# xiexh20/CHORE

Measured on AMD Instinct MI355X. Metric: query-points/sec (HGFilters encode + 20k-pt MLP field query per 512x512 image), higher is better.
Workload: dtype fp16x3; 1 GPU; BASELINE configs[1]: encode 4x(5,512,512) + query 4x20000 points per GPU per step; images_per_gpu=4, points_per_image=20000, batches_in_flight=2

## Files before the change

chore_amd/csrc/conv_mw.hip:

```cpp
#include "conv_common.h"
#include <cstdio>
#include <cstdlib>
#include <cstring>
#include <type_traits>

using namespace conv_detail;

#ifndef MW_DBG
#define MW_DBG 0
#endif

#ifdef MW_STAMPS
__device__ unsigned long long g_mw_stamps[2048 * 8];
#define MWSTAMP(i) do { if (threadIdx.x == 0 && blockIdx.x < 2048) g_mw_stamps[blockIdx.x * 8 + (i)] = wall_clock64(); } while (0)
extern "C" int chore_debug_mw_stamps(unsigned long long* out, int n) {
    return (int)hipMemcpyFromSymbol(out, HIP_SYMBOL(g_mw_stamps), sizeof(unsigned long long) * (n < 2048 * 8 ? n : 2048 * 8));
}
#else
#define MWSTAMP(i) do { } while (0)
#endif

namespace {

constexpr int PTW = 32;
constexpr int MWT = 256;

template <int TAPS, int TH_, int NT_, int TPS_, int NSLOT_, bool X3_, int WPL_> struct MGeo {
    static constexpr int TH = TH_, NT = NT_, TPS = TPS_, NSLOT = NSLOT_;
    static constexpr int PAD = (TAPS == 9) ? 1 : 0;
    static constexpr int PW = PTW + 2 * PAD, PH = TH + 2 * PAD, ROWS = PH * PW;
    static constexpr int RB = X3_ ? 144 : 80;
    static constexpr int PATCHB = (ROWS + 1) * RB;
    static constexpr int KROWS = TAPS / TPS;
    static constexpr int NB = NT / 32;
    static constexpr int SB1 = TPS * KGC * NB * 1024;
    static constexpr int SBYTES = WPL_ * SB1;
    static constexpr int NBW = NT >= 128 ? 2 : (NT == 64 ? (TH_ >= 4 ? 2 : 1) : 1);
    static constexpr int WAVES_N = NB / NBW, WAVES_M = 4 / WAVES_N, MB = TH / WAVES_M;
    static constexpr int SCR_LD = NT + 4;
    static constexpr int G8 = NT / 8;
    static constexpr int NU = TH * PTW * G8 / MWT;
    static constexpr bool CROSS = NSLOT >= 3 && KROWS > 1;
    static constexpr size_t main_bytes(int Cin) { return (size_t)2 * PATCHB + (size_t)NSLOT * SBYTES + (size_t)Cin * 8 + 16; }
    static constexpr int NROW = MWT / G8;
    static constexpr int NSEG = 4 * NT >= MWT ? 1 : MWT / (4 * NT);
    static constexpr size_t stat_bytes(int kinds) { return (size_t)(NROW + NSEG) * kinds * NT * 4; }
    static constexpr size_t scr_bytes() { return (size_t)TH * PTW * SCR_LD * 4; }
    static constexpr size_t epi_bytes() {
        size_t m = scr_bytes();
        if (stat_bytes(4) > m) m = stat_bytes(4);
        if (stat_bytes(6) > m) m = stat_bytes(6);
        return m;
    }
    static size_t smem_bytes(int Cin) { return main_bytes(Cin) > epi_bytes() ? main_bytes(Cin) : epi_bytes(); }
    static_assert(MB >= 1 && WAVES_M * MB == TH, "tile rows must divide over the waves");
    static_assert(NU >= 1, "epilogue units");
    static_assert((SBYTES / 16) % MWT == 0, "a K-step's weights: whole vectors per thread");
};

__host__ __device__ constexpr int mw_next_use(int k, int j, int UP, int KROWS, int RPS, int NVP) {
    for (int d = UP; d < KROWS; d += UP)
        if (((k + d) % KROWS) * RPS + j < NVP) return k + d;
    return k + KROWS;
}

typedef float f32x2 __attribute__((ext_vector_type(2)));
typedef _Float16 f16x2_t __attribute__((ext_vector_type(2)));
__device__ __forceinline__ unsigned cvt_pk_f16(float a, float b) {
    const f16x2_t h = {(_Float16)a, (_Float16)b};
    return __builtin_bit_cast(unsigned, h);
}
template <int HI> __device__ __forceinline__ float sub_half(float y, unsigned h) {
    float r;
    if constexpr (HI) asm("v_fma_mix_f32 %0, -%1, 1.0, %2 op_sel:[1,0,0] op_sel_hi:[1,0,0]" : "=v"(r) : "v"(h), "v"(y));
    else asm("v_fma_mix_f32 %0, -%1, 1.0, %2 op_sel:[0,0,0] op_sel_hi:[1,0,0]" : "=v"(r) : "v"(h), "v"(y));
    return r;
}

__device__ __forceinline__ void wg_barrier_mw() {
    asm volatile("s_waitcnt lgkmcnt(0)" ::: "memory");
    __builtin_amdgcn_s_barrier();
    asm volatile("" ::: "memory");
    __builtin_amdgcn_sched_barrier(0);
}

template <typename T, int TAPS, int TH_, int NT_, int TPS_, int NSLOT_, bool GN, bool SC, bool POOL = false>
__global__ __launch_bounds__(MWT, 1) void conv_mw_kernel(ConvArgs a) {
    if constexpr (IS_X3<T> || IS_H16<T>) f16_saturate_mode();
    constexpr bool BF = std::is_same<T, bf16_t>::value;
    static_assert(IS_X3<T> || IS_H16<T> || BF, "conv_mw_kernel: fp16 x 3, fp16 or bf16 operands");
    constexpr bool X3 = IS_X3<T>;
    constexpr int WPL = BF ? 1 : 2;
    using ST = typename std::conditional<X3, float, unsigned short>::type;
    constexpr int LVI = X3 ? 2 : 1;
    using G = MGeo<TAPS, TH_, NT_, TPS_, NSLOT_, X3, WPL>;
    constexpr int NSLOT = G::NSLOT;
    constexpr int TH = G::TH, NT = G::NT, TPS = G::TPS, PAD = G::PAD, PW = G::PW, ROWS = G::ROWS, RB = G::RB;
    constexpr int PATCHB = G::PATCHB, KROWS = G::KROWS, SB1 = G::SB1, SBYTES = G::SBYTES;
    constexpr int NBW = G::NBW, WAVES_N = G::WAVES_N, MB = G::MB, SCR_LD = G::SCR_LD, G8 = G::G8, NU = G::NU;
    constexpr bool CROSS = G::CROSS;
    constexpr int KGE = 16, CC = 32;
    constexpr int NTASK = ROWS * 4;
    constexpr int NVP = (NTASK + MWT - 1) / MWT;
    constexpr int RPS = KROWS > 1 ? (NVP + KROWS - 2) / (KROWS > 1 ? KROWS - 1 : 1) : NVP;
    constexpr int SVEC = SBYTES / 16, SBV = SVEC / MWT, SV1 = SB1 / 16;
    constexpr int NKS = TPS * KGC;
    constexpr int UP = KROWS == 9 ? 3 : KROWS;
    static_assert(KROWS % UP == 0 && NKS % 2 == 0, "register-set rotation / fragment double buffer");

    extern __shared__ __attribute__((aligned(16))) char smem[];
    char* patch = smem;
    char* bst = smem + 2 * PATCHB;
    float* ss_lds = (float*)(bst + NSLOT * SBYTES);

    const int tid = threadIdx.x, lane = tid & 63;
    const int wid = __builtin_amdgcn_readfirstlane(tid >> 6);
    MWSTAMP(0);
    float in_mul = 1.f, in_inv = 1.f;
    if constexpr (X3 && SC) x3_in_scale(a.in_amax, in_mul, in_inv);
    const int wn = wid % WAVES_N, wm = wid / WAVES_N;
    const int tiles_x = (a.W + PTW - 1) / PTW;
    const int ntn = a.Cout / NT, tiles = tiles_x * ((a.H + TH - 1) / TH);
    int lid = blockIdx.x;
    {
        const int nwg = gridDim.x, q = nwg >> 3, r = nwg & 7, xcd = lid & 7;
        lid = (xcd < r ? xcd * (q + 1) : r * (q + 1) + (xcd - r) * q) + (lid >> 3);
    }
    const int n_tile = lid % ntn, tileb = lid / ntn, tile = tileb % tiles, b = tileb / tiles;
    const int ty0 = (tile / tiles_x) * TH, tx0 = (tile % tiles_x) * PTW;
    const int Cin = a.in.C;
    const int NKG = Cin / KGE, NB = a.Cout / 32;
    const int NCH = Cin / CC;
    const ST* in_b = (const ST*)a.in.p + (size_t)b * a.H * a.W * a.in.cs + a.in.co;

    const int crot = (tile * 5 + n_tile * 3) % NCH;
    auto chunk_of = [&](int ci) -> int { int x = ci + crot; return x >= NCH ? x - NCH : x; };

    const int tv = tid & 3;
    int toff[NVP];
    int trow[NVP];
#pragma unroll
    for (int m = 0; m < NVP; ++m) {
        const int row = (tid >> 2) + (MWT / 4) * m;
// ... 112 lines not shown
            for (int j = 0; j < SBV; ++j) wpro[u][j] = wb[woff[j]];
        }
        __builtin_amdgcn_sched_barrier(0);
        if (tid < Cin) {
            float sc = 1.f, sh = 0.f;
            if constexpr (GN) {
                double t[2];
#pragma unroll
                for (int k = 0; k < 2; ++k) {
                    const long long top = st_hi[k] + (long long)(st_lo[k] >> 32);
                    t[k] = ((double)top * 0x1p32 + (double)(st_lo[k] & 0xffffffffull)) * 0x1p-40;
                }
                const double n = (double)(a.H * a.W) * gs_in;
                const double mean = t[0] / n;
                double var = t[1] / n - mean * mean;
                if (var < 0.0) var = 0.0;
                const float rstd = 1.0f / sqrtf((float)var + 1e-5f);
                sc = rstd * gam;
                sh = bet - (float)mean * sc;
            }
            ss_lds[4 * (tid >> 1) + (tid & 1)] = sc;
            ss_lds[4 * (tid >> 1) + 2 + (tid & 1)] = sh;
        }
#pragma unroll
        for (int m = 0; m < NVP; ++m) {
            const int row = (tid >> 2) + (MWT / 4) * m;
            if (toff[m] < 0 && row < ROWS) {
                const u32x4 z = {0u, 0u, 0u, 0u};
#pragma unroll
                for (int pbuf = 0; pbuf < 2; ++pbuf) {
                    char* d = patch + pbuf * PATCHB + row * RB + tv * 16;
                    *(u32x4*)d = z;
                    if constexpr (X3) *(u32x4*)(d + 64) = z;
                }
            }
        }
        wg_barrier_mw();
        f32x2 sc[4], sh[4];
        load_ss(sc, sh, c00);
#pragma unroll
        for (int m = 0; m < NVP; ++m) put_task(p0[m], toff[m], sc, sh, trow[m], 0);
#pragma unroll
        for (int u = 0; u < NPRO; ++u)
#pragma unroll
            for (int j = 0; j < SBV; ++j) *(u32x4*)(bst + u * SBYTES + (tid + j * MWT) * 16) = wpro[u][j];
    }

    const float ASCALE = BF ? 1.0f : (SC ? in_inv / (float)(1 << X3_WSHIFT) : 1.0f / (float)(1 << X3_WSHIFT));
    const int g8 = tid % G8;
    const int nv = n_tile * NT + g8 * 8;
    const size_t img = (size_t)b * a.H * a.W;
    const ST* res_p = a.res.p ? (const ST*)a.res.p + img * a.res.cs + a.res.co + nv : nullptr;

    u32x4 rq[NU][LVI];
    auto fetch_res = [&]() {
#pragma unroll
        for (int j = 0; j < NU; ++j) {
            const int p = (tid + MWT * j) / G8;
            const int y = ty0 + p / PTW, x = tx0 + p % PTW;
            const bool ok = (y < a.H) && (x < a.W);
            const size_t pix = (size_t)y * a.W + x;
            const u32x4 z = {0u, 0u, 0u, 0u};
#pragma unroll
            for (int k = 0; k < LVI; ++k) rq[j][k] = (res_p && ok) ? *((const u32x4*)(res_p + pix * a.res.cs) + k) : z;
        }
    };

    f32x16 acc[MB][NBW];
#pragma unroll
    for (int m = 0; m < MB; ++m)
#pragma unroll
        for (int q = 0; q < NBW; ++q)
#pragma unroll
            for (int r = 0; r < 16; ++r) acc[m][q][r] = 0.f;

    u32x4 pset[UP][RPS][LVI], wset[SBV];
    auto task_of = [&](int k, int j) -> int { return k * RPS + j; };
#pragma unroll
    for (int k = 0; k < UP; ++k)
#pragma unroll
        for (int j = 0; j < RPS; ++j)
            if (task_of(k, j) < NVP) load_task(pset[k][j], toff[task_of(k, j)], chunk_of(NCH > 1 ? 1 : 0) * CC);
    {
        constexpr int u = NSLOT - 1;
        const int uc = u / KROWS < NCH ? u / KROWS : NCH - 1;
        const u32x4* wb = w_of(uc, u % KROWS);
#pragma unroll
        for (int j = 0; j < SBV; ++j) wset[j] = wb[woff[j]];
    }
    const int half = lane >> 5, px = lane & 31;
    const char* a_ptr = patch + ((wm * MB) * PW + px) * RB + 16 * half;
    const char* b_ptr = bst + (wn * NBW) * 1024 + lane * 16;
    u32x4 af[2][MB], afl[2][MB], bf[2][NBW], bfl[2][NBW];
    auto load_frag = [&](int fs, int pbuf, int krow, int slot, int ks) {
        const char* bs = b_ptr + slot * SBYTES;
        const char* ar = a_ptr + pbuf * PATCHB + ((TPS == 3) ? (krow * PW) * RB : ((TPS == 1 && TAPS == 9) ? ((krow / 3) * PW + krow % 3) * RB : 0));
        const int t = ks / KGC, kg = ks % KGC;
        const int ky = (TPS == 9) ? t / 3 : 0, kx = (TPS == 9) ? t % 3 : t;
        if constexpr ((MW_DBG & 8) != 0) return;
#pragma unroll
        for (int q = 0; q < NBW; ++q) bf[fs][q] = *(const u32x4*)(bs + ((t * KGC + kg) * (NT / 32) + q) * 1024);
        if constexpr (X3) {
#pragma unroll
            for (int m = 0; m < MB; ++m) afl[fs][m] = *(const u32x4*)(ar + ((m + ky) * PW + kx) * RB + 64 + kg * 32);
        }
#pragma unroll
        for (int m = 0; m < MB; ++m) af[fs][m] = *(const u32x4*)(ar + ((m + ky) * PW + kx) * RB + kg * 32);
        if constexpr (WPL == 2) {
#pragma unroll
            for (int q = 0; q < NBW; ++q) bfl[fs][q] = *(const u32x4*)(bs + SB1 + ((t * KGC + kg) * (NT / 32) + q) * 1024);
        }
    };
    constexpr int NRD = (X3 ? 2 : 1) * MB + WPL * NBW, NMF = (X3 ? 3 : WPL) * MB * NBW;
    int slot = 0;
    wg_barrier_mw();
    MWSTAMP(1);
    load_frag(0, 0, 0, 0, 0);
// ... 53 lines not shown
                                                                               __builtin_bit_cast(f16x8_t, bf[ks & 1][q]), acc[m][q], 0, 0, 0);
                }
                if constexpr (BF) {
#pragma unroll
                    for (int m = 0; m < MB; ++m)
#pragma unroll
                        for (int q = 0; q < NBW; ++q)
                            acc[m][q] = __builtin_amdgcn_mfma_f32_32x32x16_bf16(__builtin_bit_cast(bf16x8_t, af[ks & 1][m]),
                                                                                __builtin_bit_cast(bf16x8_t, bf[ks & 1][q]), acc[m][q], 0, 0, 0);
                } else {
#pragma unroll
                    for (int m = 0; m < MB; ++m)
#pragma unroll
                        for (int q = 0; q < NBW; ++q)
                            acc[m][q] = __builtin_amdgcn_mfma_f32_32x32x16_f16(__builtin_bit_cast(f16x8_t, af[ks & 1][m]),
                                                                               __builtin_bit_cast(f16x8_t, bfl[ks & 1][q]), acc[m][q], 0, 0, 0);
#pragma unroll
                    for (int m = 0; m < MB; ++m)
#pragma unroll
                        for (int q = 0; q < NBW; ++q)
                            acc[m][q] = __builtin_amdgcn_mfma_f32_32x32x16_f16(__builtin_bit_cast(f16x8_t, af[ks & 1][m]),
                                                                               __builtin_bit_cast(f16x8_t, bf[ks & 1][q]), acc[m][q], 0, 0, 0);
                }
#pragma unroll
                for (int i = 0; i < NMF; ++i) {
                    __builtin_amdgcn_sched_group_barrier(0x008, 1, 0);
                    if (pre && i < NRD) __builtin_amdgcn_sched_group_barrier(0x100, 1, 0);
                    __builtin_amdgcn_sched_group_barrier(0x002, 3, 0);
                    __builtin_amdgcn_sched_group_barrier(0x020, 1, 0);
                    __builtin_amdgcn_sched_group_barrier(0x200, 1, 0);
                }
                __builtin_amdgcn_sched_barrier(0);
            }
            if constexpr ((MW_DBG & 16) == 0) wg_barrier_mw();
            if (!CROSS && !lastk) {
                load_frag(0, k + 1 < KROWS ? pb : pb ^ 1, (k + 1) % KROWS, nslot, 0);
                __builtin_amdgcn_sched_barrier(0);
            }
            slot = nslot;
        }
    };
    {
        int c = 0;
#pragma unroll 1
        for (; c + 1 < NCH; ++c) chunk_body(c, std::true_type{}, std::false_type{});
        chunk_body(c, std::false_type{}, std::true_type{});
    }

    MWSTAMP(2);
    if constexpr ((MW_DBG & 32) != 0) {
        if (a.dbg == 12345) a.bias = (const float*)&acc[0][0];
        return;
    }
    float* scr = (float*)smem;
#pragma unroll
    for (int q = 0; q < NBW; ++q) {
        const int ch = (wn * NBW + q) * 32 + px;
        const float bias = a.bias ? a.bias[n_tile * NT + ch] : 0.f;
#pragma unroll
        for (int m = 0; m < MB; ++m)
#pragma unroll
            for (int r = 0; r < 16; ++r)
                scr[((wm * MB + m) * PTW + mfma32_row(r, half)) * SCR_LD + ch] = acc[m][q][r] * ASCALE + bias;
    }
    wg_barrier_mw();
    MWSTAMP(3);

    static_assert(!POOL || (IS_X3<T> && !SC), "the pooled output: fp32 tensors of the forward pass");
    ST* out_p = (!POOL || a.out.p) ? (ST*)a.out.p + img * a.out.cs + a.out.co + nv : nullptr;
    ST* raw_p = a.raw.p ? (ST*)a.raw.p + img * a.raw.cs + a.raw.co + nv : nullptr;
    using ET = typename std::conditional<X3, float, typename std::conditional<BF, bf16_t, h16_t>::type>::type;
    constexpr bool do_pool = POOL;
    const bool want_stats = a.st_raw || a.st_out || (do_pool && a.st_pool);
    f32x2 sr[4], qr[4], so[4], qo[4];
#pragma unroll
    for (int e = 0; e < 4; ++e) { sr[e] = qr[e] = so[e] = qo[e] = f32x2{0.f, 0.f}; }
#pragma unroll
    for (int j = 0; j < NU; ++j) {
        const int p = (tid + MWT * j) / G8;
        const int y = ty0 + p / PTW, x = tx0 + p % PTW;
        float f[8];
        {
            const f32x4 lo = *(const f32x4*)(scr + p * SCR_LD + g8 * 8), hi = *(const f32x4*)(scr + p * SCR_LD + g8 * 8 + 4);
            f[0] = lo[0]; f[1] = lo[1]; f[2] = lo[2]; f[3] = lo[3]; f[4] = hi[0]; f[5] = hi[1]; f[6] = hi[2]; f[7] = hi[3];
        }
        if (y < a.H && x < a.W) {
            const size_t pix = (size_t)y * a.W + x;
            if (raw_p) {
                float g[8];
#pragma unroll
                for (int e = 0; e < 8; ++e) g[e] = f[e];
                store8<ET>((ET*)(raw_p + pix * a.raw.cs), g);
                if (want_stats) {
#pragma unroll
                    for (int e = 0; e < 4; ++e) {
                        const f32x2 v = {g[2 * e], g[2 * e + 1]};
                        sr[e] += v;
                        qr[e] = __builtin_elementwise_fma(v, v, qr[e]);
                    }
                }
            }
            if (res_p) {
#pragma unroll
                for (int k = 0; k < 4; ++k) {
                    if constexpr (X3) { f[k] += __uint_as_float(rq[j][0][k]); f[4 + k] += __uint_as_float(rq[j][LVI - 1][k]); }
                    else if constexpr (BF) {
// ... 35 lines not shown
                const int pu = tid + MWT * j;
                const int pp = pu / G8, py = pp / (PTW / 2), pxx = pp % (PTW / 2);
                const int oy = (ty0 >> 1) + py, ox = (tx0 >> 1) + pxx;
                if (pu < NPU && oy < OH && ox < OW) {
                    const float* c0 = scr + ((2 * py) * PTW + 2 * pxx) * SCR_LD + g8 * 8;
                    float v[8];
#pragma unroll
                    for (int hv = 0; hv < 2; ++hv) {
                        const f32x4 va = *(const f32x4*)(c0 + 4 * hv), vb = *(const f32x4*)(c0 + SCR_LD + 4 * hv);
                        const f32x4 vc = *(const f32x4*)(c0 + PTW * SCR_LD + 4 * hv), vd = *(const f32x4*)(c0 + (PTW + 1) * SCR_LD + 4 * hv);
                        const f32x4 r = (((va + vb) + vc) + vd) * 0.25f;
                        v[4 * hv] = r[0]; v[4 * hv + 1] = r[1]; v[4 * hv + 2] = r[2]; v[4 * hv + 3] = r[3];
                    }
                    store8<float>(pool_p + ((size_t)oy * OW + ox) * a.pool.cs, v);
#pragma unroll
                    for (int e = 0; e < 4; ++e) {
                        const f32x2 t = {v[2 * e], v[2 * e + 1]};
                        sp[e] += t;
                        qp[e] = __builtin_elementwise_fma(t, t, qp[e]);
                    }
                }
            }
        }
    }

    MWSTAMP(4);
    auto reduce_stats = [&](auto kinds_t) {
        constexpr int KINDS = decltype(kinds_t)::value;
        constexpr int RL = KINDS * NT, NROW = G::NROW, NSEG = G::NSEG, RPSEG = NROW / NSEG;
        static_assert(RPSEG * NSEG == NROW, "statistics reduction geometry");
        static_assert((size_t)(NROW + NSEG) * RL * 4 <= G::epi_bytes(), "statistics reduction scratch");
        wg_barrier_mw();
        float* part = (float*)smem;
        float* red = part + NROW * RL;
        {
            float* pr = part + (tid / G8) * RL + g8 * 8;
            auto park = [&](float* q, const f32x2 (&v)[4]) {
                *(f32x4*)q = f32x4{v[0][0], v[0][1], v[1][0], v[1][1]};
                *(f32x4*)(q + 4) = f32x4{v[2][0], v[2][1], v[3][0], v[3][1]};
            };
            park(pr, sr); park(pr + NT, qr); park(pr + 2 * NT, so); park(pr + 3 * NT, qo);
            if constexpr (KINDS == 6) { park(pr + 4 * NT, sp); park(pr + 5 * NT, qp); }
        }
        wg_barrier_mw();
        for (int cs = tid; cs < NSEG * RL; cs += MWT) {
            const int col = cs % RL, seg = cs / RL;
            const float* pc = part + (seg * RPSEG) * RL + col;
            float t = 0.f;
#pragma unroll
            for (int r = 0; r < RPSEG; ++r) t += pc[r * RL];
            red[seg * RL + col] = t;
        }
        wg_barrier_mw();
        if (tid < NT) {
            const int cg = n_tile * NT + tid;
#pragma unroll
            for (int k = 0; k < KINDS / 2; ++k) {
                GroupStat* st = k == 0 ? a.st_raw : (k == 1 ? a.st_out : a.st_pool);
                if (!st) continue;
                const int gs = (k == 0 ? a.st_raw_C : (k == 1 ? a.st_out_C : a.st_pool_C)) / GN_GROUPS;
                const int co = k == 0 ? a.st_raw_co : (k == 1 ? a.st_out_co : a.st_pool_co);
                float t1 = 0.f, t2 = 0.f;
#pragma unroll
                for (int g = 0; g < NSEG; ++g) { t1 += red[g * RL + (2 * k) * NT + tid]; t2 += red[g * RL + (2 * k + 1) * NT + tid]; }
                const float s1 = group_lane_sum(t1, gs), s2 = group_lane_sum(t2, gs);
                GroupStat* o = st + (size_t)b * GN_GROUPS + (co + cg) / gs;
                if (tid % gs == 0) stat_add(&o->sum, act_hi_cells(a.B), s1);
                if (tid % gs == (gs > 1 ? 1 : 0)) stat_add(&o->sq, act_hi_cells(a.B), s2);
            }
        }
    };
    if (want_stats) {
        reduce_stats(std::integral_constant<int, POOL ? 6 : 4>{});
    }
    MWSTAMP(5);
}

template <typename T, int TAPS, int TH, int NT, int TPS, int NSLOT, bool GN, bool SC, bool POOL = false>
int launch_mw_t(chore_handle* h, const ConvArgs& a, hipStream_t s) {
    using G = MGeo<TAPS, TH, NT, TPS, NSLOT, IS_X3<T>, std::is_same<T, bf16_t>::value ? 1 : 2>;
    size_t smem = G::smem_bytes(a.in.C);
    const size_t lds_cu = chore_lds_per_cu(h);
    if (smem > lds_cu) CHORE_FAIL(h, CHORE_EINVAL, "conv_mw: %zu bytes of LDS, the CU has %zu", smem, lds_cu);
    smem = lds_cu;
    const int tiles = ((a.W + PTW - 1) / PTW) * ((a.H + TH - 1) / TH);
    dim3 grid(tiles * (a.Cout / NT) * a.B);
    return CHORE_LAUNCH(h, s, (conv_mw_kernel<T, TAPS, TH, NT, TPS, NSLOT, GN, SC, POOL>), grid, dim3(MWT), chore_lds(smem, lds_cu), a);
}

}

int conv_mw_fill(int asked) {
    static const int env = getenv("CHORE_CONV_MW_FILL") ? atoi(getenv("CHORE_CONV_MW_FILL")) : 0;
    const int v = env > 0 ? env : asked;
    return v > 0 ? v : 256;
}
bool conv_mw_on(int dtype, int taps) {
    static const char* env = getenv("CHORE_CONV_MW");
    if (env && env[0] == '0') return false;
    return dtype == CHORE_F16X3 && taps == 9;
}
PcPlan conv_mw_plan(int dtype, int taps, int B, int H, int W, int Cin, int Cout, int fill_asked) {
    PcPlan p = conv_pc_plan(dtype, taps, B, H, W, Cin, Cout);
    static const bool th2 = getenv("CHORE_CONV_MW_TH2") != nullptr;
    if (th2 && p.th && taps == 9 && Cout % 128 == 0 && p.nt < 128 && H % 2 == 0) {
        const long tiles2 = (long)B * (H / 2) * ((W + 31) / 32) * (Cout / 128);
        if (tiles2 >= 256) { p.th = 2; p.nt = 128; p.tps = 1; p.nslot = 3; }
    }
    const int fill = conv_mw_fill(fill_asked);
    if (fill < 256 && taps == 9 && conv_mw_on(dtype, taps) && Cin % 32 == 0 && W % 32 == 0) {
        const long px8 = (long)B * ((H + 7) / 8) * (W / 32);
        if (px8 * (Cout / 32) < 256 || !p.th || (p.th == 4 && p.nt == 32) || (p.th == 8 && p.nt == 32 && px8 * (Cout / 32) < 512)) {
            static const int cand[][4] = {{8, 128, 1, 3}, {4, 128, 1, 3}, {2, 128, 1, 3}, {8, 64, 3, 2}, {4, 64, 3, 2}, {2, 64, 1, 3},
                                          {8, 32, 3, 2}, {4, 32, 9, 2}};
            for (const auto& c : cand) {
                if (Cout % c[1] || H % c[0]) continue;
                const long wgs = (long)B * (H / c[0]) * (W / 32) * (Cout / c[1]);
                if (wgs >= fill) { p.th = c[0]; p.nt = c[1]; p.tps = c[2]; p.nslot = c[3]; break; }
            }
        }
    }
    return p;
}
bool conv_mw_has(const PcPlan& p) {
    const int key = (p.th * 1000 + p.nt) * 100 + p.tps * 10 + p.nslot;
    return key == 812813 || key == 806432 || key == 803232 || key == 406432 || key == 403292 || key == 212813 || key == 412813 || key == 206413;
}
bool conv_mw_covers(int dtype, int taps, const PcPlan& p, const ConvArgs& a) {
    if (!conv_mw_on(dtype, taps) || a.res2.p) return false;
    if (a.in_st == nullptr && a.in_amax == nullptr) return false;
    if (a.in_st != nullptr && a.in_amax != nullptr) return false;
    return conv_mw_has(p);
}

bool conv_mw_pool_covers(int dtype, int taps, int Cin, int Cout, int H, int W) {
    return conv_mw_on(dtype, taps) && Cin % 32 == 0 && Cin <= 256 && Cout % 32 == 0 && H > 0 && W > 0 && H % 2 == 0 && W % 2 == 0;
}

int launch_conv_mw(chore_handle* h, int dtype, int taps, const PcPlan& p, const ConvArgs& a, hipStream_t s) {
    if (a.pool.p && ((a.H | a.W) & 1)) CHORE_FAIL(h, CHORE_EINVAL, "conv_mw: a pooled output needs even H and W (%d x %d)", a.H, a.W);
    if (!a.pool.p && !a.out.p) CHORE_FAIL(h, CHORE_EINVAL, "conv_mw: no output");
    if (a.pool.p && a.in_amax) CHORE_FAIL(h, CHORE_EINVAL, "conv_mw: no pooled output on the data-gradient kernels");
    chore_note_conv(h, CONV_FAM_MW, p.th, p.nt, p.tps, p.nslot, conv_note_flags(a), a.in.C);
    const int key = (p.th * 1000 + p.nt) * 100 + p.tps * 10 + p.nslot;
#define MW_CASE(TH, NT, TPS, NSLOT) \
    case (TH * 1000 + NT) * 100 + TPS * 10 + NSLOT:                                              \
        return a.in_amax ? launch_mw_t<x3_t, 9, TH, NT, TPS, NSLOT, false, true>(h, a, s)         \
               : (a.pool.p ? launch_mw_t<x3_t, 9, TH, NT, TPS, NSLOT, true, false, true>(h, a, s) \
                           : launch_mw_t<x3_t, 9, TH, NT, TPS, NSLOT, true, false>(h, a, s))
    switch (key) {
        MW_CASE(8, 128, 1, 3);
        MW_CASE(4, 128, 1, 3);
        MW_CASE(2, 128, 1, 3);
        MW_CASE(2, 64, 1, 3);
        MW_CASE(8, 64, 3, 2);
        MW_CASE(8, 32, 3, 2);
        MW_CASE(4, 64, 3, 2);
        MW_CASE(4, 32, 9, 2);
    }
#undef MW_CASE
    CHORE_FAIL(h, CHORE_EINVAL, "conv_mw: no kernel for taps=%d th=%d nt=%d tps=%d nslot=%d", taps, p.th, p.nt, p.tps, p.nslot);
}
```

chore_amd/csrc/enc_common.h:

```cpp
#pragma once
#include "common.h"

typedef unsigned short bf16_t;
struct h16_t { unsigned short u; };

struct x3_t { float v; };
constexpr int X3_WSHIFT = 8;
template <typename T> struct Store { using type = T; };
template <typename T> struct IsH16 { static constexpr bool value = false; };
template <> struct IsH16<h16_t> { static constexpr bool value = true; };
template <typename T> constexpr bool IS_H16 = IsH16<T>::value;
template <> struct Store<x3_t> { using type = float; };
template <typename T> struct IsX3 { static constexpr bool value = false; };
template <> struct IsX3<x3_t> { static constexpr bool value = true; };
struct x3s_t { float v; };
template <> struct Store<x3s_t> { using type = float; };
template <> struct IsX3<x3s_t> { static constexpr bool value = true; };
template <typename T> struct IsX3S { static constexpr bool value = false; };
template <> struct IsX3S<x3s_t> { static constexpr bool value = true; };
template <typename T> constexpr bool IS_X3S = IsX3S<T>::value;
template <typename T> constexpr bool IS_X3 = IsX3<T>::value;

struct View {
    void* p = nullptr;
// ... 85 lines not shown
        for (int i = 1; i < nw; ++i) v = v > lds4[i] ? v : lds4[i];
        if (v) (void)__hip_atomic_fetch_max(&cells[cell], v, __ATOMIC_RELAXED, __HIP_MEMORY_SCOPE_AGENT);
    }
}
__device__ __forceinline__ void absmax_block(const float* __restrict__ x, size_t n4, unsigned* __restrict__ cells, unsigned blk) {
    __shared__ unsigned amax_red[4];
    const u32x4* p = (const u32x4*)x;
    unsigned m = 0u;
    const size_t stride = (size_t)AMAX_CELLS * 256;
    size_t i = (size_t)blk * 256 + threadIdx.x;
    for (; i + 7 * stride < n4; i += 8 * stride) {
        u32x4 v[8];
#pragma unroll
        for (int j = 0; j < 8; ++j) v[j] = p[i + j * stride];
#pragma unroll
        for (int j = 0; j < 8; ++j)
#pragma unroll
            for (int k = 0; k < 4; ++k) { const unsigned b = v[j][k] & 0x7fffffffu; m = b > m ? b : m; }
    }
    for (; i < n4; i += stride) {
        const u32x4 v = p[i];
#pragma unroll
        for (int k = 0; k < 4; ++k) { const unsigned b = v[k] & 0x7fffffffu; m = b > m ? b : m; }
    }
#pragma unroll
    for (int o = 32; o; o >>= 1) { const unsigned w = (unsigned)__shfl_xor((int)m, o, 64); m = m > w ? m : w; }
    if ((threadIdx.x & 63) == 0) amax_red[threadIdx.x >> 6] = m;
    __syncthreads();
    if (threadIdx.x == 0) {
        for (int k = 1; k < 4; ++k) m = m > amax_red[k] ? m : amax_red[k];
        cells[blk] = m;
    }
}
#endif
int launch_absmax_f32(chore_handle* h, const float* x, size_t n, unsigned* cells, hipStream_t s);

struct ConvArgs {
    View in;
    const GroupStat* in_st;
    const float* gamma;
    const float* beta;
    const void* wpk;
    const float* bias;
    View out;
    View raw;
    View res, res2;
    int B, H, W, Cout;
    GroupStat* st_raw = nullptr; int st_raw_C = 0, st_raw_co = 0;
    GroupStat* st_out = nullptr; int st_out_C = 0, st_out_co = 0;
    View pool;
    GroupStat* st_pool = nullptr; int st_pool_C = 0, st_pool_co = 0;
    const unsigned* in_amax = nullptr;
    int fill = 0;
    unsigned long long* dbg_ticks = nullptr;
    int dbg = 0;
};

#ifdef __HIPCC__
template <typename T> struct Vec4;
template <> struct Vec4<float> {
    static __device__ __forceinline__ f32x4 ld(const float* p) { return *(const f32x4*)p; }
    static __device__ __forceinline__ void st(float* p, f32x4 v) { *(f32x4*)p = v; }
    static __device__ __forceinline__ f32x4 st_round(float* p, f32x4 v) { *(f32x4*)p = v; return v; }
};
template <> struct Vec4<bf16_t> {
    static __device__ __forceinline__ f32x4 ld(const bf16_t* p) {
        const u16x4 v = *(const u16x4*)p;
        f32x4 r = {bf2f(v[0]), bf2f(v[1]), bf2f(v[2]), bf2f(v[3])};
        return r;
    }
    static __device__ __forceinline__ void st(bf16_t* p, f32x4 v) {
        const unsigned lo = pack2bf(v[0], v[1]), hi = pack2bf(v[2], v[3]);
        *(unsigned long long*)p = (unsigned long long)lo | ((unsigned long long)hi << 32);
    }
    static __device__ __forceinline__ f32x4 st_round(bf16_t* p, f32x4 v) {
        const unsigned lo = pack2bf(v[0], v[1]), hi = pack2bf(v[2], v[3]);
        *(unsigned long long*)p = (unsigned long long)lo | ((unsigned long long)hi << 32);
        f32x4 r = {__uint_as_float(lo << 16), __uint_as_float(lo & 0xffff0000u), __uint_as_float(hi << 16),
                   __uint_as_float(hi & 0xffff0000u)};
        return r;
    }
};
template <> struct Vec4<h16_t> {
    typedef _Float16 hx4 __attribute__((ext_vector_type(4)));
    static __device__ __forceinline__ f32x4 ld(const h16_t* p) {
        const hx4 v = *(const hx4*)p;
        f32x4 r = {(float)v[0], (float)v[1], (float)v[2], (float)v[3]};
        return r;
    }
    static __device__ __forceinline__ void st(h16_t* p, f32x4 v) {
        const hx4 o = {(_Float16)v[0], (_Float16)v[1], (_Float16)v[2], (_Float16)v[3]};
        *(hx4*)p = o;
    }
    static __device__ __forceinline__ f32x4 st_round(h16_t* p, f32x4 v) {
        const hx4 o = {(_Float16)v[0], (_Float16)v[1], (_Float16)v[2], (_Float16)v[3]};
        *(hx4*)p = o;
        f32x4 r = {(float)o[0], (float)o[1], (float)o[2], (float)o[3]};
        return r;
    }
};
#endif

inline int conv_note_flags(const ConvArgs& a, bool small_grid = false) {
    return (a.in_amax ? CONV_FLAG_SCALED : 0) | (a.in_st ? CONV_FLAG_GN : 0) | (small_grid ? CONV_FLAG_SMALL_GRID : 0) |
           (a.res.p ? CONV_FLAG_RES : 0) | (a.pool.p ? CONV_FLAG_POOL : 0);
}
// ... 71 lines not shown
```

chore_amd/csrc/encoder.hip:

```cpp
#include "enc_common.h"
#include <map>
#include <memory>
#include <functional>

namespace {

size_t align_up(size_t x, size_t a) { return (x + a - 1) / a * a; }
size_t esize(int dtype) { return (dtype == CHORE_BF16 || dtype == CHORE_F16) ? 2 : 4; }
int sdt(int dtype) { return dtype == CHORE_F16X3 ? CHORE_F32 : dtype; }

struct WEntry {
    size_t off;
    size_t bytes;
    int kind;
    int taps, cin, cout;
};

struct WLayout {
    std::map<std::string, WEntry> e;
    std::vector<std::string> order;
    size_t total = 0;
    void add(const std::string& name, size_t bytes, int kind, int taps = 0, int cin = 0, int cout = 0) {
        total = align_up(total, 256);
        e[name] = WEntry{total, bytes, kind, taps, cin, cout};
// ... 261 lines not shown
        auto it = P.L.e.find(name);
        if (it == P.L.e.end()) abort();
        return it->second;
    }
    void push(std::function<void(RunCtx&)> fn) {
        Step st;
        st.kind = S_KERNEL; st.stream = cur; st.label = cur_label; st.fn = std::move(fn);
        st.klass = cur_class; st.flops = cur_flops; st.bytes = cur_bytes;
        P.steps.push_back(std::move(st));
    }
    void fork(int child) {
        if (!concurrent) return;
        const int ev = P.n_events++;
        Step a; a.kind = S_RECORD; a.stream = cur; a.event = ev; a.label = "fork";
        Step b; b.kind = S_WAIT; b.stream = child; b.event = ev; b.label = "fork";
        P.steps.push_back(a);
        P.steps.push_back(b);
        if (child + 1 > P.n_streams) P.n_streams = child + 1;
    }
    void join(int child) {
        if (!concurrent) return;
        const int ev = P.n_events++;
        Step a; a.kind = S_RECORD; a.stream = child; a.event = ev; a.label = "join";
        Step b; b.kind = S_WAIT; b.stream = cur; b.event = ev; b.label = "join";
        P.steps.push_back(a);
        P.steps.push_back(b);
    }

    void ensure_stats(Buf& x) {
        if (x.st_valid) return;
        new_stats(x);
        const Buf xb = x;
        const int HW = x.H * x.W, Bn = B;
        cur_label = "gn_stats";
        cur_class = K_GN_STATS; cur_flops = 0.0; cur_bytes = (double)B * HW * x.C * es();
        push([=](RunCtx& r) {
            if (r.rc) return;
            r.rc = launch_gn_stats(r.h, sdt(r.dtype), view(r, xb), Bn, HW, (GroupStat*)(r.stats + xb.st_off), r.s);
        });
    }

    struct ConvSpec {
        Buf in; int in_C = 0;
        std::string gn;
        std::string wname; bool bias = false;
        Buf out; int out_co = 0;
        bool has_raw = false; Buf raw; int raw_co = 0;
        bool has_res = false; Buf res; int res_co = 0;
        bool has_res2 = false; Buf res2; int res2_co = 0;
        int taps = 9, cout = 0;
        bool stat_raw = false, stat_out = false;
        bool no_out = false;
        bool has_pool = false; Buf pool; int pool_co = 0;
    };
    void conv(const ConvSpec& c) {
        const WEntry we = w(c.wname + ".weight");
        WEntry be{}, ge{}, bte{};
        if (c.bias) be = w(c.wname + ".bias");
        const bool use_gn = !c.gn.empty();
        if (use_gn) { ge = w(c.gn + ".weight"); bte = w(c.gn + ".bias"); }
        if (use_gn && (!c.in.st_valid || c.in_C != c.in.C)) abort();
        const ConvSpec cs = c;
        cur_label = "conv " + c.wname + " taps=" + std::to_string(c.taps) + " cin=" + std::to_string(c.in_C) +
                    " cout=" + std::to_string(c.cout) + " HxW=" + std::to_string(c.in.H) + "x" + std::to_string(c.in.W);
        {
            const double px = (double)B * c.in.H * c.in.W;
            cur_class = conv_class_of(dtype, c.taps, B, c.in.H, c.in.W, c.in_C, c.cout);
            cur_flops = 2.0 * c.taps * c.in_C * c.cout * px;
            cur_bytes = px * es() * (c.in_C + c.cout * ((c.no_out ? 0.0 : 1.0) + (c.has_pool ? 0.25 : 0.0) + (c.has_raw ? 1 : 0) + (c.has_res ? 1 : 0) + (c.has_res2 ? 1 : 0)));
        }
        const int Bn = B;
        push([=](RunCtx& r) {
            if (r.rc) return;
            ConvArgs a{};
            a.fill = CONV_MW_FILL_INFER;
            a.in = view(r, cs.in, 0, cs.in_C);
            if (use_gn) {
                a.in_st = (const GroupStat*)(r.stats + cs.in.st_off);
                a.gamma = (const float*)(r.arena + ge.off);
                a.beta = (const float*)(r.arena + bte.off);
            }
            a.wpk = r.arena + we.off;
            a.bias = cs.bias ? (const float*)(r.arena + be.off) : nullptr;
            if (!cs.no_out) a.out = view(r, cs.out, cs.out_co, cs.cout);
            if (cs.has_pool) {
                a.pool = view(r, cs.pool, cs.pool_co, cs.cout);
                a.st_pool = (GroupStat*)(r.stats + cs.pool.st_off); a.st_pool_C = cs.pool.C; a.st_pool_co = cs.pool_co;
            }
            if (cs.has_raw) a.raw = view(r, cs.raw, cs.raw_co, cs.cout);
            if (cs.has_res) a.res = view(r, cs.res, cs.res_co, cs.cout);
            if (cs.has_res2) a.res2 = view(r, cs.res2, cs.res2_co, cs.cout);
            a.B = Bn; a.H = cs.in.H; a.W = cs.in.W; a.Cout = cs.cout;
            if (cs.stat_raw) {
                a.st_raw = (GroupStat*)(r.stats + cs.raw.st_off); a.st_raw_C = cs.raw.C; a.st_raw_co = cs.raw_co;
            }
            if (cs.stat_out) {
                a.st_out = (GroupStat*)(r.stats + cs.out.st_off); a.st_out_C = cs.out.C; a.st_out_co = cs.out_co;
            }
            r.rc = launch_conv(r.h, r.dtype, cs.taps, a, r.s);
        });
    }

    Buf conv_block(Buf& x, const std::string& n, int cin, int cout, bool out_unread = false, Buf* pool = nullptr, bool keep_out = true) {
        const int H = x.H, W = x.W;
        ensure_stats(x);
        Buf out = alloc(H, W, cout);
        Buf o1 = alloc(H, W, cout / 2), o2 = alloc(H, W, cout / 4);
        const bool fold = pool_fold && pool && conv_pool_covers(dtype, 9, cin, cout / 2, H, W) &&
                          conv_pool_covers(dtype, 9, cout / 2, cout / 4, H, W) && conv_pool_covers(dtype, 9, cout / 4, cout / 4, H, W);
        const bool st_out = !(pool_fold && (out_unread || (fold && !keep_out)));
        const bool wr_out = !(fold && !keep_out);
        if (fold) new_stats(*pool);
        if (st_out) new_stats(out);
        new_stats(o1);
        new_stats(o2);
        Buf res = x;
        if (cin != cout) {
            ConvSpec d;
            d.in = x; d.in_C = cin; d.gn = n + ".bn4"; d.wname = n + ".downsample.2";
            d.out = out; d.taps = 1; d.cout = cout;
            conv(d);
            res = out;
        }
        ConvSpec c1;
        c1.in = x; c1.in_C = cin; c1.gn = n + ".bn1"; c1.wname = n + ".conv1";
        c1.out = out; c1.out_co = 0; c1.has_raw = true; c1.raw = o1; c1.has_res = true; c1.res = res; c1.res_co = 0;
        c1.cout = cout / 2; c1.stat_raw = true; c1.stat_out = st_out; c1.no_out = !wr_out;
        if (fold) { c1.has_pool = true; c1.pool = *pool; c1.pool_co = 0; }
        conv(c1);
        ConvSpec c2;
        c2.in = o1; c2.in_C = cout / 2; c2.gn = n + ".bn2"; c2.wname = n + ".conv2";
        c2.out = out; c2.out_co = cout / 2; c2.has_raw = true; c2.raw = o2; c2.has_res = true; c2.res = res;
        c2.res_co = cout / 2; c2.cout = cout / 4; c2.stat_raw = true; c2.stat_out = st_out; c2.no_out = !wr_out;
        if (fold) { c2.has_pool = true; c2.pool = *pool; c2.pool_co = cout / 2; }
        conv(c2);
        ConvSpec c3;
        c3.in = o2; c3.in_C = cout / 4; c3.gn = n + ".bn3"; c3.wname = n + ".conv3";
        c3.out = out; c3.out_co = 3 * cout / 4; c3.has_res = true; c3.res = res; c3.res_co = 3 * cout / 4;
        c3.cout = cout / 4; c3.stat_out = st_out; c3.no_out = !wr_out;
        if (fold) { c3.has_pool = true; c3.pool = *pool; c3.pool_co = 3 * cout / 4; }
        conv(c3);
        release(o1);
        release(o2);
        return out;
    }

    Buf pool2(const Buf& x, const Buf* out_opt = nullptr) {
        Buf y = out_opt ? *out_opt : alloc(x.H / 2, x.W / 2, x.C);
        new_stats(y);
        cur_label = "avgpool2";
        cur_class = K_POOL; cur_flops = 0.0; cur_bytes = (double)B * x.H * x.W * x.C * es() * 1.25;
        const int Bn = B;
        push([=](RunCtx& r) {
            if (r.rc) return;
            r.rc = launch_avgpool2(r.h, sdt(r.dtype), view(r, x), view(r, y), Bn, x.H, x.W,
                                   (GroupStat*)(r.stats + y.st_off), r.s);
        });
        return y;
    }
    void upadd(Buf& a, const Buf& low) {
        cur_label = "upadd";
        cur_class = K_UPADD; cur_flops = 0.0; cur_bytes = (double)B * low.H * low.W * low.C * es() * 9.0;
        new_stats(a);
        const Buf ab = a;
        const int Bn = B;
        push([=](RunCtx& r) {
            if (r.rc) return;
            r.rc = launch_upadd(r.h, sdt(r.dtype), view(r, ab), view(r, low), view(r, ab), Bn, low.H, low.W,
                                (GroupStat*)(r.stats + ab.st_off), r.s);
        });
    }

    Buf hourglass(Buf& x, const std::string& n, int level, Buf* pooled_x = nullptr) {
        const std::string l = std::to_string(level);
        const int child = P.cfg.num_hourglass - level + 1;
        ensure_stats(x);
        const int parent = cur;
        fork(child);
        Buf pooled = !pooled_x ? pool2(x) : (pooled_x->st_valid ? *pooled_x : pool2(x, pooled_x));
        Buf low1, low2;
        if (level > 1) {
            Buf pooled1 = alloc(pooled.H / 2, pooled.W / 2, 256);
            low1 = conv_block(pooled, n + ".b2_" + l, 256, 256, false, &pooled1);
            release(pooled);
            low2 = hourglass(low1, n, level - 1, &pooled1);
        } else {
            low1 = conv_block(pooled, n + ".b2_" + l, 256, 256);
            release(pooled);
            low2 = conv_block(low1, n + ".b2_plus_" + l, 256, 256);
        }
        release(low1);
        Buf low3 = conv_block(low2, n + ".b3_" + l, 256, 256, true);
        release(low2);
// ... 369 lines not shown
```

Baseline: 20.25 million points/s.

## Add direct register-to-global epilogue for fp16x3 multi-wave conv kernel

Adds a DIRECT epilogue variant that writes accumulator fragments straight from registers to global memory, adds bias and the residual loaded in the MFMA fragment layout, and accumulates GroupNorm statistics in registers. The statistics are reduced with a permlane32 swap plus a small LDS hand-over. This skips the LDS scratch staging and the segmented stats reduction of the old epilogue, and it becomes the default for non-pooled fp16x3 launches. The trade-off is uncoalesced, strided per-lane global stores and residual loads instead of vectorized 16-byte rows. Blocks followed by a separate pool stay on the LDS path.

Result: no change. 20.42 million points/s, median of 6 (+0.8%).

```diff
diff --git a/chore_amd/csrc/conv_mw.hip b/chore_amd/csrc/conv_mw.hip
--- a/chore_amd/csrc/conv_mw.hip
+++ b/chore_amd/csrc/conv_mw.hip
@@ -52,7 +52,12 @@
         if (stat_bytes(6) > m) m = stat_bytes(6);
         return m;
     }
-    static size_t smem_bytes(int Cin) { return main_bytes(Cin) > epi_bytes() ? main_bytes(Cin) : epi_bytes(); }
+    static constexpr size_t hand_bytes() { return (size_t)WAVES_M * 4 * NT * 4; }
+    static size_t smem_bytes(int Cin, bool direct) {
+        const size_t e = direct ? hand_bytes() : epi_bytes();
+        return main_bytes(Cin) > e ? main_bytes(Cin) : e;
+    }
+    static_assert(hand_bytes() <= (size_t)2 * PATCHB, "statistics hand-over fits the patch buffers");
     static_assert(MB >= 1 && WAVES_M * MB == TH, "tile rows must divide over the waves");
     static_assert(NU >= 1, "epilogue units");
     static_assert((SBYTES / 16) % MWT == 0, "a K-step's weights: whole vectors per thread");
@@ -84,11 +89,12 @@
     __builtin_amdgcn_sched_barrier(0);
 }
 
-template <typename T, int TAPS, int TH_, int NT_, int TPS_, int NSLOT_, bool GN, bool SC, bool POOL = false>
+template <typename T, int TAPS, int TH_, int NT_, int TPS_, int NSLOT_, bool GN, bool SC, bool POOL = false, bool DIRECT = false>
 __global__ __launch_bounds__(MWT, 1) void conv_mw_kernel(ConvArgs a) {
     if constexpr (IS_X3<T> || IS_H16<T>) f16_saturate_mode();
     constexpr bool BF = std::is_same<T, bf16_t>::value;
     static_assert(IS_X3<T> || IS_H16<T> || BF, "conv_mw_kernel: fp16 x 3, fp16 or bf16 operands");
+    static_assert(!DIRECT || (IS_X3<T> && !POOL), "the direct epilogue: fp32 tensors, no pooled output (a 2x2 window straddles waves)");
     constexpr bool X3 = IS_X3<T>;
     constexpr int WPL = BF ? 1 : 2;
     using ST = typename std::conditional<X3, float, unsigned short>::type;
@@ -307,17 +313,46 @@
     const size_t img = (size_t)b * a.H * a.W;
     const ST* res_p = a.res.p ? (const ST*)a.res.p + img * a.res.cs + a.res.co + nv : nullptr;
 
+    const int dhalf = lane >> 5, dpx = lane & 31;
+    const int dch = n_tile * NT + wn * NBW * 32 + dpx;
+    const int dxlim = a.W - tx0 - 4 * dhalf;
+    const bool tile_full = (ty0 + TH <= a.H) && (tx0 + PTW <= a.W);
+
     u32x4 rq[NU][LVI];
+    f32x2 rqd[DIRECT ? MB : 1][NBW][8];
     auto fetch_res = [&]() {
-#pragma unroll
-        for (int j = 0; j < NU; ++j) {
-            const int p = (tid + MWT * j) / G8;
-            const int y = ty0 + p / PTW, x = tx0 + p % PTW;
-            const bool ok = (y < a.H) && (x < a.W);
-            const size_t pix = (size_t)y * a.W + x;
-            const u32x4 z = {0u, 0u, 0u, 0u};
-#pragma unroll
-            for (int k = 0; k < LVI; ++k) rq[j][k] = (res_p && ok) ? *((const u32x4*)(res_p + pix * a.res.cs) + k) : z;
+        if constexpr (DIRECT) {
+            if (!a.res.p) return;
+            const float* res_d = (const float*)a.res.p + img * a.res.cs + a.res.co;
+            const unsigned off = (unsigned)(4 * dhalf * a.res.cs + dch);
+            auto rows = [&](auto full_t) {
+                constexpr bool FULL = decltype(full_t)::value;
+#pragma unroll
+                for (int m = 0; m < MB; ++m) {
+                    const int y = ty0 + wm * MB + m;
+                    const bool yok = FULL || y < a.H;
+#pragma unroll
+                    for (int r = 0; r < 16; ++r) {
+                        const float* rowp = res_d + ((size_t)y * a.W + tx0 + mfma32_row(r, 0)) * a.res.cs;
+                        const bool ok = yok && (FULL || mfma32_row(r, 0) < dxlim);
+#pragma unroll
+                        for (int q = 0; q < NBW; ++q) rqd[m][q][r >> 1][r & 1] = ok ? rowp[off + q * 32] : 0.f;
+                    }
+                }
+            };
+            if (tile_full) rows(std::true_type{});
+            else rows(std::false_type{});
+        } else {
+#pragma unroll
+            for (int j = 0; j < NU; ++j) {
+                const int p = (tid + MWT * j) / G8;
+                const int y = ty0 + p / PTW, x = tx0 + p % PTW;
+                const bool ok = (y < a.H) && (x < a.W);
+                const size_t pix = (size_t)y * a.W + x;
+                const u32x4 z = {0u, 0u, 0u, 0u};
+#pragma unroll
+                for (int k = 0; k < LVI; ++k) rq[j][k] = (res_p && ok) ? *((const u32x4*)(res_p + pix * a.res.cs) + k) : z;
+            }
         }
     };
 
@@ -477,6 +512,117 @@
         if (a.dbg == 12345) a.bias = (const float*)&acc[0][0];
         return;
     }
+    auto finish_stats = [&](const float* red, auto kinds_t, auto npart_t) {
+        constexpr int KINDS = decltype(kinds_t)::value, NPART = decltype(npart_t)::value, RL = KINDS * NT;
+        if (tid < NT) {
+            const int cg = n_tile * NT + tid;
+#pragma unroll
+            for (int k = 0; k < KINDS / 2; ++k) {
+                GroupStat* st = k == 0 ? a.st_raw : (k == 1 ? a.st_out : a.st_pool);
+                if (!st) continue;
+                const int gs = (k == 0 ? a.st_raw_C : (k == 1 ? a.st_out_C : a.st_pool_C)) / GN_GROUPS;
+                const int co = k == 0 ? a.st_raw_co : (k == 1 ? a.st_out_co : a.st_pool_co);
+                float t1 = 0.f, t2 = 0.f;
+#pragma unroll
+                for (int g = 0; g < NPART; ++g) { t1 += red[g * RL + (2 * k) * NT + tid]; t2 += red[g * RL + (2 * k + 1) * NT + tid]; }
+                const float s1 = group_lane_sum(t1, gs), s2 = group_lane_sum(t2, gs);
+                GroupStat* o = st + (size_t)b * GN_GROUPS + (co + cg) / gs;
+                if (tid % gs == 0) stat_add(&o->sum, act_hi_cells(a.B), s1);
+                if (tid % gs == (gs > 1 ? 1 : 0)) stat_add(&o->sq, act_hi_cells(a.B), s2);
+            }
+        }
+    };
+
+    if constexpr (DIRECT) {
+        MWSTAMP(3);
+        float* out_d = (float*)a.out.p + img * a.out.cs + a.out.co;
+        float* raw_d = a.raw.p ? (float*)a.raw.p + img * a.raw.cs + a.raw.co : nullptr;
+        const unsigned out_off = (unsigned)(4 * dhalf * a.out.cs + dch), raw_off = (unsigned)(4 * dhalf * a.raw.cs + dch);
+        const bool want_stats = a.st_raw || a.st_out;
+        const bool with_res = a.res.p != nullptr;
+        f32x2 bias2[NBW];
+#pragma unroll
+        for (int q = 0; q < NBW; ++q) {
+            const float bq = a.bias ? a.bias[dch + q * 32] : 0.f;
+            bias2[q] = f32x2{bq, bq};
+        }
+        f32x2 sr[NBW], qr[NBW], so[NBW], qo[NBW];
+#pragma unroll
+        for (int q = 0; q < NBW; ++q) sr[q] = qr[q] = so[q] = qo[q] = f32x2{0.f, 0.f};
+        auto rows = [&](auto full_t) {
+            constexpr bool FULL = decltype(full_t)::value;
+            auto put = [&](float* base, int cs, unsigned off, int m, int y, f32x2 (&s)[NBW], f32x2 (&sq)[NBW]) {
+#pragma unroll
+                for (int r = 0; r < 16; ++r) {
+                    float* rowp = base + ((size_t)y * a.W + tx0 + mfma32_row(r, 0)) * cs;
+                    if (FULL || mfma32_row(r, 0) < dxlim) {
+#pragma unroll
+                        for (int q = 0; q < NBW; ++q) rowp[off + q * 32] = acc[m][q][r];
+                    }
+                }
+                if (want_stats) {
+#pragma unroll
+                    for (int q = 0; q < NBW; ++q)
+#pragma unroll
+                        for (int r = 0; r < 16; r += 2) {
+                            f32x2 v = {acc[m][q][r], acc[m][q][r + 1]};
+                            if constexpr (!FULL) {
+                                v[0] = mfma32_row(r, 0) < dxlim ? v[0] : 0.f;
+                                v[1] = mfma32_row(r + 1, 0) < dxlim ? v[1] : 0.f;
+                            }
+                            s[q] += v;
+                            sq[q] = __builtin_elementwise_fma(v, v, sq[q]);
+                        }
+                }
+            };
+#pragma unroll
+            for (int m = 0; m < MB; ++m) {
+                const int y = ty0 + wm * MB + m;
+                if (!FULL && y >= a.H) continue;
+#pragma unroll
+                for (int q = 0; q < NBW; ++q)
+#pragma unroll
+                    for (int r = 0; r < 16; r += 2) {
+                        f32x2 v = {acc[m][q][r], acc[m][q][r + 1]};
+                        v = v * ASCALE + bias2[q];
+                        acc[m][q][r] = v[0]; acc[m][q][r + 1] = v[1];
+                    }
+                if (raw_d) put(raw_d, a.raw.cs, raw_off, m, y, sr, qr);
+                if (with_res) {
+#pragma unroll
+                    for (int q = 0; q < NBW; ++q)
+#pragma unroll
+                        for (int r = 0; r < 16; r += 2) {
+                            acc[m][q][r] += rqd[m][q][r >> 1][0];
+                            acc[m][q][r + 1] += rqd[m][q][r >> 1][1];
+                        }
+                }
+                put(out_d, a.out.cs, out_off, m, y, so, qo);
+            }
+        };
+        if (tile_full) rows(std::true_type{});
+        else rows(std::false_type{});
+        MWSTAMP(4);
+        if (want_stats) {
+            float* hand = (float*)smem;
+            auto halves = [&](const f32x2& v) -> float {
+                const float t = v[0] + v[1];
+                const auto x = __builtin_amdgcn_permlane32_swap(__float_as_uint(t), __float_as_uint(t), false, false);
+                return __uint_as_float(x[0]) + __uint_as_float(x[1]);
+            };
+#pragma unroll
+            for (int q = 0; q < NBW; ++q) {
+                const float t0 = halves(sr[q]), t1 = halves(qr[q]), t2 = halves(so[q]), t3 = halves(qo[q]);
+                float* hp = hand + (wm * 4) * NT + (wn * NBW + q) * 32 + dpx;
+                if (dhalf == 0) { hp[0] = t0; hp[NT] = t1; hp[2 * NT] = t2; hp[3 * NT] = t3; }
+            }
+            wg_barrier_mw();
+            finish_stats(hand, std::integral_constant<int, 4>{}, std::integral_constant<int, G::WAVES_M>{});
+        }
+        MWSTAMP(5);
+        return;
+    }
+
     float* scr = (float*)smem;
 #pragma unroll
     for (int q = 0; q < NBW; ++q) {
@@ -618,23 +764,7 @@
             red[seg * RL + col] = t;
         }
         wg_barrier_mw();
-        if (tid < NT) {
-            const int cg = n_tile * NT + tid;
-#pragma unroll
-            for (int k = 0; k < KINDS / 2; ++k) {
-                GroupStat* st = k == 0 ? a.st_raw : (k == 1 ? a.st_out : a.st_pool);
-                if (!st) continue;
-                const int gs = (k == 0 ? a.st_raw_C : (k == 1 ? a.st_out_C : a.st_pool_C)) / GN_GROUPS;
-                const int co = k == 0 ? a.st_raw_co : (k == 1 ? a.st_out_co : a.st_pool_co);
-                float t1 = 0.f, t2 = 0.f;
-#pragma unroll
-                for (int g = 0; g < NSEG; ++g) { t1 += red[g * RL + (2 * k) * NT + tid]; t2 += red[g * RL + (2 * k + 1) * NT + tid]; }
-                const float s1 = group_lane_sum(t1, gs), s2 = group_lane_sum(t2, gs);
-                GroupStat* o = st + (size_t)b * GN_GROUPS + (co + cg) / gs;
-                if (tid % gs == 0) stat_add(&o->sum, act_hi_cells(a.B), s1);
-                if (tid % gs == (gs > 1 ? 1 : 0)) stat_add(&o->sq, act_hi_cells(a.B), s2);
-            }
-        }
+        finish_stats(red, kinds_t, std::integral_constant<int, NSEG>{});
     };
     if (want_stats) {
         reduce_stats(std::integral_constant<int, POOL ? 6 : 4>{});
@@ -642,16 +772,16 @@
     MWSTAMP(5);
 }
 
-template <typename T, int TAPS, int TH, int NT, int TPS, int NSLOT, bool GN, bool SC, bool POOL = false>
+template <typename T, int TAPS, int TH, int NT, int TPS, int NSLOT, bool GN, bool SC, bool POOL = false, bool DIRECT = false>
 int launch_mw_t(chore_handle* h, const ConvArgs& a, hipStream_t s) {
     using G = MGeo<TAPS, TH, NT, TPS, NSLOT, IS_X3<T>, std::is_same<T, bf16_t>::value ? 1 : 2>;
-    size_t smem = G::smem_bytes(a.in.C);
+    size_t smem = G::smem_bytes(a.in.C, DIRECT);
     const size_t lds_cu = chore_lds_per_cu(h);
     if (smem > lds_cu) CHORE_FAIL(h, CHORE_EINVAL, "conv_mw: %zu bytes of LDS, the CU has %zu", smem, lds_cu);
     smem = lds_cu;
     const int tiles = ((a.W + PTW - 1) / PTW) * ((a.H + TH - 1) / TH);
     dim3 grid(tiles * (a.Cout / NT) * a.B);
-    return CHORE_LAUNCH(h, s, (conv_mw_kernel<T, TAPS, TH, NT, TPS, NSLOT, GN, SC, POOL>), grid, dim3(MWT), chore_lds(smem, lds_cu), a);
+    return CHORE_LAUNCH(h, s, (conv_mw_kernel<T, TAPS, TH, NT, TPS, NSLOT, GN, SC, POOL, DIRECT>), grid, dim3(MWT), chore_lds(smem, lds_cu), a);
 }
 
 }
@@ -666,6 +796,14 @@
     if (env && env[0] == '0') return false;
     return dtype == CHORE_F16X3 && taps == 9;
 }
+enum { MW_EPI_TABLE = 0, MW_EPI_LDS = 1, MW_EPI_DIRECT = 2 };
+static int conv_mw_epi() {
+    static const char* env = getenv("CHORE_CONV_MW_EPI");
+    if (env && !strcmp(env, "lds")) return MW_EPI_LDS;
+    if (env && !strcmp(env, "direct")) return MW_EPI_DIRECT;
+    return MW_EPI_TABLE;
+}
+static constexpr bool mw_direct_default(int , int , int , int ) { return true; }
 PcPlan conv_mw_plan(int dtype, int taps, int B, int H, int W, int Cin, int Cout, int fill_asked) {
     PcPlan p = conv_pc_plan(dtype, taps, B, H, W, Cin, Cout);
     static const bool th2 = getenv("CHORE_CONV_MW_TH2") != nullptr;
@@ -709,11 +847,17 @@
     if (a.pool.p && a.in_amax) CHORE_FAIL(h, CHORE_EINVAL, "conv_mw: no pooled output on the data-gradient kernels");
     chore_note_conv(h, CONV_FAM_MW, p.th, p.nt, p.tps, p.nslot, conv_note_flags(a), a.in.C);
     const int key = (p.th * 1000 + p.nt) * 100 + p.tps * 10 + p.nslot;
+    const int epi = conv_mw_epi();
 #define MW_CASE(TH, NT, TPS, NSLOT) \
-    case (TH * 1000 + NT) * 100 + TPS * 10 + NSLOT:                                              \
-        return a.in_amax ? launch_mw_t<x3_t, 9, TH, NT, TPS, NSLOT, false, true>(h, a, s)         \
-               : (a.pool.p ? launch_mw_t<x3_t, 9, TH, NT, TPS, NSLOT, true, false, true>(h, a, s) \
-                           : launch_mw_t<x3_t, 9, TH, NT, TPS, NSLOT, true, false>(h, a, s))
+    case (TH * 1000 + NT) * 100 + TPS * 10 + NSLOT: {                                                                   \
+        const bool direct = !a.lds_epi && (epi == MW_EPI_DIRECT || (epi == MW_EPI_TABLE && mw_direct_default(TH, NT, TPS, NSLOT))); \
+        if (a.pool.p) return launch_mw_t<x3_t, 9, TH, NT, TPS, NSLOT, true, false, true>(h, a, s);                       \
+        if (a.in_amax)                                                                                                   \
+            return direct ? launch_mw_t<x3_t, 9, TH, NT, TPS, NSLOT, false, true, false, true>(h, a, s)                  \
+                          : launch_mw_t<x3_t, 9, TH, NT, TPS, NSLOT, false, true>(h, a, s);                              \
+        return direct ? launch_mw_t<x3_t, 9, TH, NT, TPS, NSLOT, true, false, false, true>(h, a, s)                      \
+                      : launch_mw_t<x3_t, 9, TH, NT, TPS, NSLOT, true, false>(h, a, s);                                  \
+    }
     switch (key) {
         MW_CASE(8, 128, 1, 3);
         MW_CASE(4, 128, 1, 3);
diff --git a/chore_amd/csrc/enc_common.h b/chore_amd/csrc/enc_common.h
--- a/chore_amd/csrc/enc_common.h
+++ b/chore_amd/csrc/enc_common.h
@@ -161,6 +161,7 @@
     GroupStat* st_pool = nullptr; int st_pool_C = 0, st_pool_co = 0;
     const unsigned* in_amax = nullptr;
     int fill = 0;
+    bool lds_epi = false;
     unsigned long long* dbg_ticks = nullptr;
     int dbg = 0;
 };
diff --git a/chore_amd/csrc/encoder.hip b/chore_amd/csrc/encoder.hip
--- a/chore_amd/csrc/encoder.hip
+++ b/chore_amd/csrc/encoder.hip
@@ -337,6 +337,7 @@
         bool stat_raw = false, stat_out = false;
         bool no_out = false;
         bool has_pool = false; Buf pool; int pool_co = 0;
+        bool lds_epi = false;
     };
     void conv(const ConvSpec& c) {
         const WEntry we = w(c.wname + ".weight");
@@ -376,6 +377,7 @@
             if (cs.has_res) a.res = view(r, cs.res, cs.res_co, cs.cout);
             if (cs.has_res2) a.res2 = view(r, cs.res2, cs.res2_co, cs.cout);
             a.B = Bn; a.H = cs.in.H; a.W = cs.in.W; a.Cout = cs.cout;
+            a.lds_epi = cs.lds_epi;
             if (cs.stat_raw) {
                 a.st_raw = (GroupStat*)(r.stats + cs.raw.st_off); a.st_raw_C = cs.raw.C; a.st_raw_co = cs.raw_co;
             }
@@ -412,18 +414,21 @@
         c1.out = out; c1.out_co = 0; c1.has_raw = true; c1.raw = o1; c1.has_res = true; c1.res = res; c1.res_co = 0;
         c1.cout = cout / 2; c1.stat_raw = true; c1.stat_out = st_out; c1.no_out = !wr_out;
         if (fold) { c1.has_pool = true; c1.pool = *pool; c1.pool_co = 0; }
+        c1.lds_epi = pool && !fold;
         conv(c1);
         ConvSpec c2;
         c2.in = o1; c2.in_C = cout / 2; c2.gn = n + ".bn2"; c2.wname = n + ".conv2";
         c2.out = out; c2.out_co = cout / 2; c2.has_raw = true; c2.raw = o2; c2.has_res = true; c2.res = res;
         c2.res_co = cout / 2; c2.cout = cout / 4; c2.stat_raw = true; c2.stat_out = st_out; c2.no_out = !wr_out;
         if (fold) { c2.has_pool = true; c2.pool = *pool; c2.pool_co = cout / 2; }
+        c2.lds_epi = pool && !fold;
         conv(c2);
         ConvSpec c3;
         c3.in = o2; c3.in_C = cout / 4; c3.gn = n + ".bn3"; c3.wname = n + ".conv3";
         c3.out = out; c3.out_co = 3 * cout / 4; c3.has_res = true; c3.res = res; c3.res_co = 3 * cout / 4;
         c3.cout = cout / 4; c3.stat_out = st_out; c3.no_out = !wr_out;
         if (fold) { c3.has_pool = true; c3.pool = *pool; c3.pool_co = 3 * cout / 4; }
+        c3.lds_epi = pool && !fold;
         conv(c3);
         release(o1);
         release(o2);
```
